# richardbaihe/a3t

Hardware: AMD Instinct MI355X
Metric: mel-frames/sec (train) (higher is better)
Workload: dtype bf16; 1 GPU; VCTK A3T masked-mel train step: 6+6 Conformer blocks d=384 H=2 ff=1536(k3), B=32/GPU, T_mel=1000, T_phn=120, postnet 5x256x5, fwd+bwd+clip+Adam, dropout 0.2/0.2/0.2 + postnet 0.5 (recipe); global_batch=32, parallelism=dp1, params=100799808

## Files before the change

a3t_amd/_lib.py:

```python
import ctypes
import os
from ctypes import POINTER, c_char_p, c_float, c_int, c_int32, c_int64, c_void_p

import torch

HERE = os.path.dirname(os.path.abspath(__file__))
LIB_PATH = os.environ.get("A3T_LIB_PATH") or os.path.join(HERE, "lib", "liba3t_hip.so")

F32, BF16 = 0, 1
ACT_NONE, ACT_RELU, ACT_TANH, ACT_SWISH = 0, 1, 2, 3
ACC_STORE, ACC_ADD, ACC_ATOMIC, ACC_SOLE = 0, 1, 2, 3


class GemmDesc(ctypes.Structure):
    _fields_ = [
        ("A", c_void_p), ("B", c_void_p), ("C", c_void_p), ("bias", c_void_p), ("R", c_void_p), ("S", c_void_p),
        ("M", c_int32), ("N", c_int32), ("K", c_int32),
        ("a_rs", c_int64), ("a_cs", c_int64),
        ("b_rs", c_int64), ("b_cs", c_int64), ("b_ts", c_int64),
        ("c_rs", c_int64),
        ("batch", c_int32), ("batch_inner", c_int32),
        ("a_bs0", c_int64), ("a_bs1", c_int64), ("b_bs0", c_int64), ("b_bs1", c_int64),
        ("c_bs0", c_int64), ("c_bs1", c_int64),
        ("taps", c_int32), ("pad", c_int32), ("dil", c_int32), ("Tseq", c_int32), ("kshift", c_int32),
        ("alpha", c_float),
        ("act", c_int32), ("accumulate", c_int32), ("splitk", c_int32),
        ("a_dtype", c_int32), ("b_dtype", c_int32), ("c_dtype", c_int32), ("compute", c_int32),
        ("s_dtype", c_int32), ("colsum_slots", c_int32),
        ("colsum", c_void_p), ("colsum_bs1", c_int64), ("colsum_scale", c_float), ("drop_key", ctypes.c_uint32),
        ("drop_p", c_float), ("colsum_ss", c_int32),
        ("keep_out", c_void_p), ("keep_in", c_void_p),
        ("a_signmask", c_int32), ("keep_layout", c_int32),
        ("A2", c_void_p), ("B2", c_void_p), ("b2_cs", c_int64), ("b2_bs0", c_int64), ("b2_bs1", c_int64), ("colsum2", c_void_p),
        ("a2_rs", c_int64), ("a_unaligned", c_int32),
    ]


_P = c_void_p
_SIGS = {
    "a3t_gemm": [POINTER(GemmDesc), _P],
    "a3t_gemm_plan": [POINTER(GemmDesc), c_char_p, c_int],
    "a3t_layernorm_fwd": [_P, _P, _P, _P, c_int, _P, _P, c_int, c_int, c_float, _P],
    "a3t_layernorm_bwd": [_P, c_int, _P, _P, _P, _P, _P, _P, _P, _P, _P, _P, c_float, c_int, c_int, c_float,
                          ctypes.c_uint32, _P],
    "a3t_col_reduce": [_P, c_int, _P, _P, _P, _P, c_int, c_int, c_int64, c_int, _P],
    "a3t_f64_to_f32_add": [_P, _P, c_int, c_float, _P],
    "a3t_bn_act_fwd": [_P, _P, _P, _P, _P, _P, _P, _P, _P, c_int, c_int, c_int, c_float, c_float, c_int, c_int, _P],
    "a3t_bn_act_bwd_a": [_P, c_int, _P, _P, _P, _P, _P, _P, c_int, c_int, c_int, _P],
    "a3t_bn_act_bwd_b": [_P, c_int, _P, _P, _P, _P, _P, _P, _P, _P, _P, c_int, c_int, c_int, c_int, _P],
    "a3t_glu_dwconv_fwd": [_P, c_int, _P, _P, _P, c_int, _P, c_int, c_int, c_int, c_int, _P],
    "a3t_glu_dwconv_bwd": [_P, _P, c_int, _P, c_int, _P, _P, c_int, _P, _P, _P, c_int, c_int, c_int, c_int, _P],
    "a3t_add_pos_bias": [_P, _P, _P, _P, _P, c_int, c_int, c_int, _P],
    "a3t_add_pos_bias_bwd": [_P, _P, _P, c_int, c_int, c_int, _P],
    "a3t_relpos_softmax_fwd": [_P, _P, c_int, _P, _P, c_int, c_int, c_int, c_int, c_int64, c_int64, c_int64, c_float, _P,
                               c_float, ctypes.c_uint32, _P],
    "a3t_relpos_softmax_bwd": [_P, c_int, _P, c_int, _P, _P, c_int, c_int, c_int, c_int, c_int64, c_int64, c_int64, c_float, _P,
                               c_float, c_int64, c_int64, ctypes.c_uint32, _P, _P],
    "a3t_attn_fwd_train": [_P, _P, _P, _P, _P, _P, _P, _P, _P, _P, _P, c_int, c_int, c_int, c_int, c_int64, c_int64, c_int64,
                           c_int64, c_float, c_float, ctypes.c_uint32, _P, _P, _P],
    "a3t_attn_scale_rows": [_P, _P, _P, c_int, c_int, c_int, c_int, _P],
    "a3t_attn_bwd_ds": [_P, _P, _P, _P, _P, _P, _P, c_int, c_int, c_int, c_int, c_int64, c_int64, c_int64, c_int64, c_float,
                        c_float, ctypes.c_uint32, c_int, c_int64, _P],
    "a3t_attn_fwd": [_P, _P, _P, _P, _P, _P, _P, _P, c_int, c_int, c_int, c_int, c_int64, c_int64, c_int64, c_int64,
                     c_float, c_float, ctypes.c_uint32, _P, _P, _P],
    "a3t_pwg_block": [_P, _P, _P, _P, _P, _P, _P, _P, c_int, c_int, c_int, _P],
    "a3t_mask_fill": [_P, _P, _P, _P, c_int, c_int, c_int, _P],
    "a3t_embed_finish_fwd": [_P, _P, _P, _P, _P, _P, _P, c_int, c_int, c_int, c_int, c_float, c_float, ctypes.c_uint32,
                             _P, _P],
    "a3t_embed_finish_bwd": [_P, _P, _P, _P, _P, _P, _P, _P, c_int, c_int, c_int, c_int, c_int, c_int, c_float, c_float,
                             ctypes.c_uint32, _P],
    "a3t_scale": [_P, _P, c_int64, c_float, _P],
    "a3t_axpy": [_P, _P, c_int64, c_float, _P],
    "a3t_attn_bias_fold": [_P, c_int32, c_int32, _P, _P, _P, _P],
    "a3t_scale_dev": [_P, _P, c_int64, _P, _P],
    "a3t_slice_rows": [_P, _P, c_int, c_int, c_int, c_int, c_int, c_int, _P],
    "a3t_cast_bf16": [_P, _P, c_int64, _P],
    "a3t_cast_bf16_conv_t": [_P, _P, _P, _P, c_int, c_int, c_int, c_int, _P],
    "a3t_split_bf16": [_P, _P, _P, c_int64, _P],
    "a3t_reflect_pad": [_P, _P, c_int, c_int, c_int, c_int, _P],
    "a3t_stft_amp": [_P, _P, c_int64, c_int, c_int, _P],
    "a3t_logmel_finish": [_P, _P, c_int, c_int, c_int, _P],
    "a3t_mlm_loss": [_P, _P, _P, _P, _P, _P, _P, _P, c_int, c_int, c_int, c_float, _P],
    "a3t_mlm_loss_scratch_floats": [c_int],
    "a3t_sumsq": [_P, c_int64, _P, _P],
# ... 68 lines not shown
```

a3t_amd/build.py:

```python
import os
import subprocess
import sys
from concurrent.futures import ThreadPoolExecutor

HERE = os.path.dirname(os.path.abspath(__file__))
CSRC = os.path.join(HERE, "csrc")
LIBDIR = os.path.join(HERE, "lib")
LIB = os.path.join(LIBDIR, "liba3t_hip.so")
SOURCES = ["gemm.hip", "gemm_bf16.hip", "gemm_bf16_8p.hip", "gemm_bf16_pn.hip", "gemm_bf16_tt.hip", "attn_fused.hip", "norm_reduce.hip", "convmod_attn.hip", "dwconv_vec.hip", "misc.hip", "pwg_fused.hip", "features.hip", "duration.hip"]
FLAGS = ["--offload-arch=gfx950", "-O3", "-std=c++17", "-fPIC", "-ffp-contract=off"] + os.environ.get("A3T_EXTRA_FLAGS", "").split()


RES_SOURCES = ("gemm_bf16.hip", "gemm_bf16_8p.hip", "gemm_bf16_pn.hip", "gemm_bf16_tt.hip", "attn_fused.hip", "norm_reduce.hip")
RES_FLAG = ["-Rpass-analysis=kernel-resource-usage"]


def _save_resources(report, path):
    import json
    import re
    cur, rows = None, {}
    for ln in report.splitlines():
        m = re.search(r"Function Name: (\S+)", ln)
        if m:
            cur = m.group(1)
            rows[cur] = {}
            continue
        m = re.search(r"remark:\s+([\w \[\]/]+?): (\d+)", ln)
        if m and cur:
            rows[cur][m.group(1).strip()] = int(m.group(2))
    with open(path, "w") as f:
        json.dump(rows, f, indent=1)


def _hipcc():
    for c in ("/opt/rocm/bin/hipcc", "hipcc"):
        if os.path.exists(c) or c == "hipcc":
            return c


def _stale(out, deps):
    if not os.path.exists(out):
        return True
    t = os.path.getmtime(out)
    return any(os.path.getmtime(d) > t for d in deps)


# ... 34 lines not shown
```

a3t_amd/csrc/convmod_attn.hip:

```cpp
#include <hip/hip_runtime.h>
#include <stdint.h>
#include "../../include/a3t_hip.h"
#include "dtype_io.h"

#define WAVE 64
__device__ __forceinline__ float sigm(float v) { return 1.f / (1.f + __expf(-v)); }
__device__ __forceinline__ float bf2f_(unsigned int h) { return __uint_as_float(h << 16); }
__device__ __forceinline__ float wsum(float v) {
#pragma unroll
    for (int o = 32; o > 0; o >>= 1) v += __shfl_xor(v, o, WAVE);
    return v;
}
__device__ __forceinline__ float wmax(float v) {
#pragma unroll
    for (int o = 32; o > 0; o >>= 1) v = fmaxf(v, __shfl_xor(v, o, WAVE));
    return v;
}

#define DW_TT 64
#define DW_KMAX 31

template <int KT>
__global__ __launch_bounds__(256) void glu_dwconv_fwd_kernel(const void* __restrict__ g, int g_dt,
                                                             const float* __restrict__ wdw,
// ... 33 lines not shown
    for (int k = 0; k < KT; ++k) w[k] = (k < K) ? wdw[(int64_t)c * K + k] : 0.f;
    const float bias = bdw[c];
    if (K == KT) {
        for (int r0 = ty * 4; r0 < DW_TT; r0 += 16) {
            float v[KT + 3];
#pragma unroll
            for (int j = 0; j < KT + 3; ++j) v[j] = win[r0 + j][tx];
#pragma unroll
            for (int tt = 0; tt < 4; ++tt) {
                float acc = bias;
#pragma unroll
                for (int k = 0; k < KT; ++k) acc += w[k] * v[tt + k];
                int t = t0 + r0 + tt;
                if (t < Tseq) z[(mbase + t) * (int64_t)C + c] = acc;
            }
        }
        return;
    }
    for (int r = ty; r < DW_TT; r += 4) {
        int t = t0 + r;
        if (t >= Tseq) break;
        float acc = bias;
#pragma unroll
        for (int k = 0; k < KT; ++k)
            if (k < K) acc += w[k] * win[r + k][tx];
        z[(mbase + t) * (int64_t)C + c] = acc;
    }
}

int a3t_glu_dwconv_fwd_vec(const void* g, const float* wdw, const float* bdw, void* glu, float* z, int M, int C, int K,
                           int Tseq, hipStream_t stream);
int a3t_glu_dwconv_bwd_vec(const float* dz, const void* g, const void* glu, const float* wdw, void* dg, float* dwdw,
                           float* dbdw, float* dg_colsum, int M, int C, int K, int Tseq, hipStream_t stream);
static inline bool dw_al16(const void* p) { return ((uintptr_t)p & 15) == 0; }

extern "C" int a3t_glu_dwconv_fwd(const void* g, int g_dtype, const float* wdw, const float* bdw, void* glu,
                                  int glu_dtype, float* z, int M, int C, int K, int Tseq, void* stream) {
    if (K > DW_KMAX || (K & 1) == 0 || Tseq <= 0 || M % Tseq) return A3T_EINVAL;
    if (g_dtype == A3T_BF16 && glu_dtype == A3T_BF16 && C % 64 == 0 && dw_al16(g) && dw_al16(glu) && dw_al16(z))
        return a3t_glu_dwconv_fwd_vec(g, wdw, bdw, glu, z, M, C, K, Tseq, (hipStream_t)stream);
    int B = M / Tseq, tiles_t = (Tseq + DW_TT - 1) / DW_TT;
    dim3 grid((C + 63) / 64, B * tiles_t);
    if (K <= 7)
        hipLaunchKernelGGL(glu_dwconv_fwd_kernel<7>, grid, dim3(256), 0, (hipStream_t)stream, g, g_dtype, wdw, bdw, glu,
                           glu_dtype, z, C, K, Tseq, tiles_t);
    else if (K <= 15)
        hipLaunchKernelGGL(glu_dwconv_fwd_kernel<15>, grid, dim3(256), 0, (hipStream_t)stream, g, g_dtype, wdw, bdw, glu,
                           glu_dtype, z, C, K, Tseq, tiles_t);
    else
        hipLaunchKernelGGL(glu_dwconv_fwd_kernel<DW_KMAX>, grid, dim3(256), 0, (hipStream_t)stream, g, g_dtype, wdw, bdw,
                           glu, glu_dtype, z, C, K, Tseq, tiles_t);
    return (int)hipGetLastError();
}

template <int KT>
__global__ __launch_bounds__(256, 3) void glu_dwconv_bwd_kernel(const float* __restrict__ dz, const void* __restrict__ g,
                                                             int g_dt, const void* __restrict__ glu, int glu_dt,
                                                             const float* __restrict__ wdw, void* __restrict__ dg,
                                                             int dg_dt, float* dwdw, float* dbdw, float* dgsum, int C,
                                                             int K, int Tseq, int tiles_t, int tiles_per_block,
                                                             int chunks) {
    __shared__ float wdz[DW_TT + DW_KMAX - 1][64];
    __shared__ float wgl[DW_TT + DW_KMAX - 1][64];
    __shared__ float red[4][64];
    const int tx = threadIdx.x & 63, ty = threadIdx.x >> 6;
    const int c = blockIdx.x * 64 + tx;
// ... 134 lines not shown
        red[ty][tx] = sgb;
        __syncthreads();
        if (ty == 0 && c < C) atomicAdd(&dgsum[C + c], red[0][tx] + red[1][tx] + red[2][tx] + red[3][tx]);
    }
}

extern "C" int a3t_glu_dwconv_bwd(const float* dz, const void* g, int g_dtype, const void* glu, int glu_dtype,
                                  const float* wdw, void* dg, int dg_dtype, float* dwdw, float* dbdw, float* dg_colsum,
                                  int M, int C, int K, int Tseq, void* stream) {
    if (K > DW_KMAX || (K & 1) == 0 || Tseq <= 0 || M % Tseq) return A3T_EINVAL;
    if (g_dtype == A3T_BF16 && glu_dtype == A3T_BF16 && dg_dtype == A3T_BF16 && C % 64 == 0 && dw_al16(g) &&
        dw_al16(glu) && dw_al16(dg) && dw_al16(dz))
        return a3t_glu_dwconv_bwd_vec(dz, g, glu, wdw, dg, dwdw, dbdw, dg_colsum, M, C, K, Tseq, (hipStream_t)stream);
    int B = M / Tseq, tiles_t = (Tseq + DW_TT - 1) / DW_TT;
    int cb = (C + 63) / 64;
    int chunks = 1;
    while (cb * B * chunks < 1024 && chunks < tiles_t) ++chunks;
    int tpb = (tiles_t + chunks - 1) / chunks;
    chunks = (tiles_t + tpb - 1) / tpb;
    dim3 grid(cb, B * chunks);
#define DWB(KT)                                                                                                       \
    hipLaunchKernelGGL(glu_dwconv_bwd_kernel<KT>, grid, dim3(256), 0, (hipStream_t)stream, dz, g, g_dtype, glu, glu_dtype, \
                       wdw, dg, dg_dtype, dwdw, dbdw, dg_colsum, C, K, Tseq, tiles_t, tpb, chunks)
    if (K <= 7)
        DWB(7);
    else if (K <= 15)
        DWB(15);
    else
        DWB(DW_KMAX);
#undef DWB
    return (int)hipGetLastError();
}

__global__ void add_pos_bias_kernel(const void* __restrict__ qkv, const float* __restrict__ bu,
                                    const float* __restrict__ bv, void* __restrict__ qu, void* __restrict__ qv,
                                    int dt, int64_t n, int d) {
    for (int64_t i = (int64_t)blockIdx.x * blockDim.x + threadIdx.x; i < n; i += (int64_t)gridDim.x * blockDim.x) {
        int64_t m = i / d;
        int c = (int)(i - m * d);
        float q = ldx(qkv, dt, m * 3 * d + c);
        stx(qu, dt, i, q + bu[c]);
        stx(qv, dt, i, q + bv[c]);
    }
}
__device__ __forceinline__ void apb_unpack8(const uint4& u, float* f) {
    f[0] = bf2f_(u.x & 0xffff), f[1] = bf2f_(u.x >> 16), f[2] = bf2f_(u.y & 0xffff), f[3] = bf2f_(u.y >> 16);
    f[4] = bf2f_(u.z & 0xffff), f[5] = bf2f_(u.z >> 16), f[6] = bf2f_(u.w & 0xffff), f[7] = bf2f_(u.w >> 16);
}
__device__ __forceinline__ uint4 apb_pack8(const float* f) {
    uint4 u;
    u.x = io_pack2(f[0], f[1]), u.y = io_pack2(f[2], f[3]);
    u.z = io_pack2(f[4], f[5]), u.w = io_pack2(f[6], f[7]);
    return u;
}
__global__ void add_pos_bias_bf16_kernel(const unsigned short* __restrict__ qkv, const float* __restrict__ bu,
                                         const float* __restrict__ bv, unsigned short* __restrict__ qu,
                                         unsigned short* __restrict__ qv, int64_t n8, int d8) {
    for (int64_t i = (int64_t)blockIdx.x * blockDim.x + threadIdx.x; i < n8; i += (int64_t)gridDim.x * blockDim.x) {
        const int64_t m = i / d8;
        const int c = (int)(i - m * d8) * 8;
        float q[8], o[8];
        apb_unpack8(*(const uint4*)(qkv + m * 3 * d8 * 8 + c), q);
        const float4 u0 = *(const float4*)(bu + c), u1 = *(const float4*)(bu + c + 4);
        const float4 v0 = *(const float4*)(bv + c), v1 = *(const float4*)(bv + c + 4);
        const float uu[8] = {u0.x, u0.y, u0.z, u0.w, u1.x, u1.y, u1.z, u1.w};
        const float vv[8] = {v0.x, v0.y, v0.z, v0.w, v1.x, v1.y, v1.z, v1.w};
// ... 468 lines not shown
```

a3t_amd/csrc/dwconv_vec.hip:

```cpp
#include <hip/hip_runtime.h>
#include <stdint.h>
#include "../../include/a3t_hip.h"
#include "dtype_io.h"

#define DW_TT 64
#define DW_KMAX 31
typedef unsigned short u16;

__device__ __forceinline__ float dv_sigm(float v) { return 1.f / (1.f + __expf(-v)); }
__device__ __forceinline__ float dv_bf(unsigned int h) { return __uint_as_float(h << 16); }
__device__ __forceinline__ void dv_unpack8(const uint4& u, float* f) {
    f[0] = dv_bf(u.x & 0xffff), f[1] = dv_bf(u.x >> 16), f[2] = dv_bf(u.y & 0xffff), f[3] = dv_bf(u.y >> 16);
    f[4] = dv_bf(u.z & 0xffff), f[5] = dv_bf(u.z >> 16), f[6] = dv_bf(u.w & 0xffff), f[7] = dv_bf(u.w >> 16);
}
__device__ __forceinline__ uint4 dv_pack8(const float* f) {
    uint4 u;
    u.x = io_pack2(f[0], f[1]), u.y = io_pack2(f[2], f[3]);
    u.z = io_pack2(f[4], f[5]), u.w = io_pack2(f[6], f[7]);
    return u;
}

template <int KT>
__global__ __launch_bounds__(256) void glu_dwconv_fwd_vec_kernel(const u16* __restrict__ g, const float* __restrict__ wdw,
                                                                 const float* __restrict__ bdw, u16* __restrict__ glu,
// ... 59 lines not shown
            for (int k = 0; k < KT; ++k)
                if (k < K) acc += w[k] * win[r + k][tx];
            zt[r][tx] = acc;
        }
    }
    __syncthreads();
    {
        const int rr = tid >> 4, c4 = (tid & 15) * 4;
#pragma unroll
        for (int ps = 0; ps < 4; ++ps) {
            const int r = ps * 16 + rr, t = t0 + r;
            if (t < Tseq) *(float4*)(z + (mbase + t) * (int64_t)C + cblk + c4) = *(const float4*)&zt[r][c4];
        }
    }
}

int a3t_glu_dwconv_fwd_vec(const void* g, const float* wdw, const float* bdw, void* glu, float* z, int M, int C, int K,
                           int Tseq, hipStream_t stream) {
    const int B = M / Tseq, tiles_t = (Tseq + DW_TT - 1) / DW_TT;
    dim3 grid(C / 64, B * tiles_t);
#define DWF(KT)                                                                                                         \
    hipLaunchKernelGGL(glu_dwconv_fwd_vec_kernel<KT>, grid, dim3(256), 0, stream, (const u16*)g, wdw, bdw, (u16*)glu, z, \
                       C, K, Tseq, tiles_t)
    if (K <= 7)
        DWF(7);
    else if (K <= 15)
        DWF(15);
    else
        DWF(DW_KMAX);
#undef DWF
    return (int)hipGetLastError();
}

template <int KT>
__global__ __launch_bounds__(256, 3) void glu_dwconv_bwd_vec_kernel(const float* __restrict__ dz, const u16* __restrict__ g,
                                                                    const u16* __restrict__ glu,
                                                                    const float* __restrict__ wdw, u16* __restrict__ dg,
                                                                    float* dwdw, float* dbdw, float* dgsum, int C, int K,
                                                                    int Tseq, int tiles_t, int tiles_per_block,
                                                                    int chunks) {
    __shared__ __attribute__((aligned(16))) float wdz[DW_TT + DW_KMAX - 1][64];
    __shared__ __attribute__((aligned(16))) u16 wgl[DW_TT + DW_KMAX - 1][64];
    __shared__ __attribute__((aligned(16))) u16 gt[2][DW_TT][64];
    __shared__ float red[4][64];
    const int tid = threadIdx.x, tx = tid & 63, ty = tid >> 6;
    const int cblk = blockIdx.x * 64, c = cblk + tx;
    const int b = blockIdx.y / chunks, tile0 = (blockIdx.y % chunks) * tiles_per_block;
    const int pad = (K - 1) / 2;
    const int64_t mbase = (int64_t)b * Tseq;
    const int rows = DW_TT + K - 1;
    float w[KT], dw[KT];
#pragma unroll
    for (int k = 0; k < KT; ++k) {
        w[k] = (k < K) ? wdw[(int64_t)c * K + k] : 0.f;
        dw[k] = 0.f;
    }
    float db = 0.f, sga = 0.f, sgb = 0.f;
    for (int tile = tile0; tile < min(tiles_t, tile0 + tiles_per_block); ++tile) {
        const int t0 = tile * DW_TT;
        __syncthreads();
        {
            const int r16 = tid >> 4, c4 = (tid & 15) * 4;
            const int r32 = tid >> 3, c8 = (tid & 7) * 8;
            float4 vz[6];
            uint4 vg[3], va[2], vb[2];
#pragma unroll
            for (int ps = 0; ps < 6; ++ps) {
                const int r = ps * 16 + r16, t = t0 - pad + r;
                const bool ok = (r < rows) && (t >= 0) && (t < Tseq);
                vz[ps] = *(const float4*)(dz + (ok ? (mbase + t) * (int64_t)C + cblk + c4 : 0));
                if (!ok) vz[ps] = make_float4(0.f, 0.f, 0.f, 0.f);
            }
#pragma unroll
            for (int ps = 0; ps < 3; ++ps) {
                const int r = ps * 32 + r32, t = t0 - pad + r;
                const bool ok = (r < rows) && (t >= 0) && (t < Tseq);
                vg[ps] = *(const uint4*)(glu + (ok ? (mbase + t) * (int64_t)C + cblk + c8 : 0));
                if (!ok) vg[ps] = make_uint4(0, 0, 0, 0);
            }
#pragma unroll
            for (int ps = 0; ps < 2; ++ps) {
                const int r = ps * 32 + r32, t = t0 + r;
                const bool ok = t < Tseq;
                const u16* src = g + (ok ? (mbase + t) * (int64_t)(2 * C) + cblk + c8 : 0);
                va[ps] = *(const uint4*)src;
                vb[ps] = *(const uint4*)(src + (ok ? C : 0));
            }
#pragma unroll
            for (int ps = 0; ps < 6; ++ps) {
                const int r = ps * 16 + r16;
                if (r < rows) *(float4*)&wdz[r][c4] = vz[ps];
            }
#pragma unroll
            for (int ps = 0; ps < 3; ++ps) {
// ... 75 lines not shown
                if (t < Tseq) {
                    u16* dst = dg + (mbase + t) * (int64_t)(2 * C) + cblk + c8;
                    *(uint4*)dst = *(const uint4*)&gt[0][r][c8];
                    *(uint4*)(dst + C) = *(const uint4*)&gt[1][r][c8];
                }
            }
        }
    }
    __syncthreads();
    float* part = &wdz[0][0];
    for (int i = tid; i < 64 * K; i += 256) part[i] = 0.f;
    __syncthreads();
#pragma unroll
    for (int k = 0; k < KT; ++k)
        if (k < K) atomicAdd(&part[tx * K + k], dw[k]);
    __syncthreads();
    for (int i = tid; i < 64 * K; i += 256) atomicAdd(&dwdw[(int64_t)cblk * K + i], part[i]);
    __syncthreads();
    red[ty][tx] = db;
    __syncthreads();
    if (ty == 0) atomicAdd(&dbdw[c], red[0][tx] + red[1][tx] + red[2][tx] + red[3][tx]);
    if (dgsum) {
        __syncthreads();
        red[ty][tx] = sga;
        __syncthreads();
        if (ty == 0) atomicAdd(&dgsum[c], red[0][tx] + red[1][tx] + red[2][tx] + red[3][tx]);
        __syncthreads();
        red[ty][tx] = sgb;
        __syncthreads();
        if (ty == 0) atomicAdd(&dgsum[C + c], red[0][tx] + red[1][tx] + red[2][tx] + red[3][tx]);
    }
}

int a3t_glu_dwconv_bwd_vec(const float* dz, const void* g, const void* glu, const float* wdw, void* dg, float* dwdw,
                           float* dbdw, float* dg_colsum, int M, int C, int K, int Tseq, hipStream_t stream) {
    const int B = M / Tseq, tiles_t = (Tseq + DW_TT - 1) / DW_TT;
    const int cb = C / 64;
    int chunks = 1;
    while (cb * B * chunks < 640 && chunks < tiles_t) ++chunks;
    const int tpb = (tiles_t + chunks - 1) / chunks;
    chunks = (tiles_t + tpb - 1) / tpb;
    dim3 grid(cb, B * chunks);
#define DWB(KT)                                                                                                       \
    hipLaunchKernelGGL(glu_dwconv_bwd_vec_kernel<KT>, grid, dim3(256), 0, stream, dz, (const u16*)g, (const u16*)glu, \
                       wdw, (u16*)dg, dwdw, dbdw, dg_colsum, C, K, Tseq, tiles_t, tpb, chunks)
    if (K <= 7)
        DWB(7);
    else if (K <= 15)
        DWB(15);
    else
        DWB(DW_KMAX);
#undef DWB
    return (int)hipGetLastError();
}
```

a3t_amd/engine.py:

```python
import math
import os
import zlib
from typing import Dict

import torch

from . import ops
from ._lib import ACC_ADD, ACC_ATOMIC, ACC_STORE, ACT_NONE, ACT_RELU, ACT_SWISH, ACT_TANH, BF16, F32
from .config import A3TConfig
from .params import ParamStore


def legacy_pe_table(c: A3TConfig) -> torch.Tensor:
    d = c.adim
    position = torch.arange(c.max_len - 1, -1, -1.0, dtype=torch.float32).unsqueeze(1)
    div = torch.exp(torch.arange(0, d, 2, dtype=torch.float32) * -(math.log(10000.0) / d))
    pe = torch.zeros(c.max_len, d)
    pe[:, 0::2] = torch.sin(position * div)
    pe[:, 1::2] = torch.cos(position * div)
    return pe


_STREAMS = {}

# ... 95 lines not shown
        self.c = cfg
        self.dropping = bool(dropout and training)
        self.step_seed = 0
        self.store = store
        self.dev = store.device
        self.ws = Workspace(self.dev)
        self.bf16 = (compute == "bf16")
        self.adt = torch.bfloat16 if self.bf16 else torch.float32
        self.cmp = BF16 if self.bf16 else F32
        self.training = training
        self.pe = legacy_pe_table(cfg).to(self.dev)
        self.sv = {}
        self.scratch64 = torch.zeros(4 * max(cfg.ff, 3 * cfg.adim, cfg.postnet_chans, 64), dtype=torch.float64,
                                     device=self.dev)
        self.bn_momentum = 0.1
        self.side = self.side2 = None
        if self.dev.type == "cuda" and os.environ.get("A3T_SIDE_STREAM", "1") != "0":
            self.side = shared_stream(self.dev, "side")
            self.side2 = (shared_stream(self.dev, "side2", high=True)
                          if os.environ.get("A3T_SIDE2", "1") != "0" else self.side)
        self._owned = {}
        self._par = 0
        self._depth = max(2, int(os.environ.get("A3T_SIDE_DEPTH", "48")))
        self._side_ev = [None] * self._depth
        self._wg_group = 4 if (self.bf16 and self.side is not None and self._depth >= 8 and
                               os.environ.get("A3T_WGRAD_GROUP", "1") != "0") else 1
        self._wg_pending = []
        self._wg_slots = set()
        self._gm_ready = None
        self._arena = {k: dict(buf=None, used=0, slots={}, dtype=dt) for k, dt in
                       (("fwd64", torch.float64), ("bwd64", torch.float64), ("bwd32", torch.float32))}
        self.colsum_slots = 16
        self.fuse_ln_dropout = True
        self.post_f32_first = os.environ.get("A3T_POST_F32_FIRST", "1") != "0"
        self.sfc_f32 = True
        self.attn_regen = True
        self.attn_bwd_ds = os.environ.get("A3T_ATTN_BWD_DS", "1") != "0"
        self.attn_signed = os.environ.get("A3T_ATTN_SIGNED", "1") != "0"
        self.attn_dq_dual = os.environ.get("A3T_ATTN_DQ_DUAL", "1") != "0"
        self.attn_dbd_view = os.environ.get("A3T_ATTN_DBD_VIEW", "1") != "0"
        self.attn_dk_main = os.environ.get("A3T_ATTN_DK_MAIN", "1") != "0"
        fa = os.environ.get("A3T_FUSED_ATTN", "auto")
        if fa not in ("auto", "fwd", "0"):
            raise ValueError(f"A3T_FUSED_ATTN={fa!r}: expected auto, fwd or 0 (the flash backward behind '1' left the library in "
                             "round 5, tools/experiments/attn_flash_backward.patch)")
        self.fused_attn_fwd_only = self.bf16 and fa == "fwd"
        self.fused_attn_auto = self.bf16 and fa == "auto"
        self.fused_attn_train = self.bf16 and fa == "auto" and os.environ.get("A3T_FUSED_ATTN_TRAIN", "1") != "0"
        self.fused_attn_train_min = 1 if os.environ.get("A3T_FUSED_ATTN_TRAIN", "1") == "2" else 64
        self._fused_now = False
        self._fused_train_now = False
        self._need_grad = training
        self._mode_tag = None
        if self.bf16:
            for n, v in (("adim", cfg.adim), ("ff", cfg.ff), ("idim", cfg.idim), ("odim", cfg.odim),
                         ("dk", cfg.dk), ("postnet_chans", cfg.postnet_chans or 8)):
                if v % 8:
                    raise ValueError(f"compute='bf16' needs {n} % 8 == 0 (16-byte DMA granules), got {v}")
            self.flat16 = torch.zeros(store.total, dtype=torch.bfloat16, device=self.dev)
            self.p16 = {k: self.flat16[o:o + math.prod(s)].view(s) for k, (o, s) in store.offsets.items()}
        self._ffn_plans = {}
        self._lin_plans = {}
        self._wt = {}
        self._late_cast = self._pos_ahead = True
        self._P_ahead, self._pos_ev = {}, None
        self._cast_ev = self._wt_ev = None
# ... 521 lines not shown
        sums = self._arena_slot("bwd64", tag + ".bnsums", 2 * C)
        ops.bn_act_bwd(dy, z, mean, rstd, p[pre + ".g"], p[pre + ".b"], sums, dz, gr[pre + ".g"], gr[pre + ".b"],
                       self.training, act, zero=False)

    def _conv_fwd(self, tag, pre, x, T):
        p, c = self.store.p, self.c
        M, d = x.shape
        cmp = self.cmp
        y = self._ln_fwd(tag + ".ln", x, pre + ".ln")
        g2 = self._act(tag + ".g", (M, 2 * d))
        ops.linear_fwd(y, self.W(pre + ".pw1"), g2, bias=p[pre + ".pb1"], compute=cmp)
        glu = self._act(tag + ".glu", (M, d))
        z = self.ws.get(tag + ".z", (M, d))
        ops.glu_dwconv_fwd(g2, p[pre + ".dw"], p[pre + ".db"], glu, z, T)
        s = self._act(tag + ".s", (M, d))
        self._bn_fwd(tag, z, pre + ".bn", pre + ".bn", ACT_SWISH, s)
        xo = self.ws.get(tag + ".xo", (M, d))
        ops.linear_fwd(s, self.W(pre + ".pw2"), xo, bias=p[pre + ".pb2"], R=x, compute=cmp,
                       drop=self._drop(c.dropout_rate, tag + ".o"))
        self.sv[tag] = (y, g2, glu, s)
        return xo

    def _conv_bwd(self, tag, pre, g, T, nb=None, nxt=None):
        p, gr, c = self.store.p, self.store.g, self.c
        M, d = g.shape
        cmp = self.cmp
        y, g2, glu, s = self.sv[tag]
        self._sub_begin()
        g16 = self._g16(g)
        ga = self._gm(g, tag + ".o", c.dropout_rate, gr[pre + ".pb2"], 1.0)
        self._lin_wgrad(ga, s, gr[pre + ".pw2"])
        ds = self.ws.get("tmp.ds", (M, d))
        self._lin_dgrad(ga, pre + ".pw2", ds)
        dz = self.ws.get("tmp.dz", (M, d))
        self._bn_bwd(tag, ds, pre + ".bn", ACT_SWISH, dz)
        dg = self._act(self._t("tmp.dg"), (M, 2 * d))
        ops.glu_dwconv_bwd(dz, g2, glu, p[pre + ".dw"], dg, gr[pre + ".dw"], gr[pre + ".db"], T,
                           dgsum=gr[pre + ".pb1"])
        self._lin_wgrad(dg, y, gr[pre + ".pw1"])
        dy = self._act("tmp.dy", (M, d))
        self._lin_dgrad(dg, pre + ".pw1", dy)
        self._pre_ln(ga, g, g16)
        self._ln_bwd(tag + ".ln", dy, pre + ".ln", g, g, g16, nb, nxt)
        self._sub_end()
        return g

    def block_fwd(self, pre, x, pos, keymask, B, T):
        x = self._ffn_fwd(pre + ".ffm", pre + ".ffm", x, T)
        x = self._mha_fwd(pre + ".mha", pre + ".mha", x, pos, keymask, B, T)
        x = self._conv_fwd(pre + ".cnv", pre + ".cnv", x, T)
        x = self._ffn_fwd(pre + ".ff", pre + ".ff", x, T)
        return self._ln_fwd(pre + ".fin", x, pre + ".fin.ln", out_dtype=torch.float32)

    def block_bwd(self, pre, g, B, T):
        gr = self.store.g
        self._ln_bwd(pre + ".fin", g, pre + ".fin.ln", None, g, self._g16(g), (gr[pre + ".ff.b2"], 0.5), pre + ".ff.o")
        self._ffn_bwd(pre + ".ff", pre + ".ff", g, T, (gr[pre + ".cnv.pb2"], 1.0), pre + ".cnv.o")
        self._conv_bwd(pre + ".cnv", pre + ".cnv", g, T, (gr[pre + ".mha.bo"], 1.0), pre + ".mha.o")
        self._mha_bwd(pre + ".mha", pre + ".mha", g, B, T, (gr[pre + ".ffm.b2"], 0.5), pre + ".ffm.o")
        self._ffn_bwd(pre + ".ffm", pre + ".ffm", g, T, None)
        return g

    def forward(self, batch: Dict[str, torch.Tensor], need_grad: bool = True, gscale: float = 1.0):
        c, p, ws = self.c, self.store.p, self.ws
        speech = batch["speech"].contiguous()
        B, Tm, idim = speech.shape
        text = batch["text"].contiguous()
        Tp = text.shape[1]
        T = Tm + Tp
        d = c.adim
        if self.bf16 and (T % 8 or Tm % 8):
# ... 229 lines not shown
```

a3t_amd/ops.py:

```python
import ctypes
import os

import torch

from . import _lib as L
from ._lib import ACC_ADD, ACC_ATOMIC, ACC_SOLE, ACC_STORE, ACT_NONE, ACT_RELU, ACT_SWISH, ACT_TANH, BF16, F32

__all__ = ["gemm", "gemm_plan", "linear_fwd", "linear_bwd_data", "linear_bwd_weight", "conv_fwd", "conv_bwd_data",
           "conv_bwd_weight"]


PROFILE = None


def _stream():
    return ctypes.c_void_p(torch.cuda.current_stream().cuda_stream)


def _ptr(t):
    if t is None:
        return None
    return ctypes.c_void_p(t.data_ptr())


# ... 239 lines not shown


def bn_act_fwd(z, stats, g, b, rmean, rvar, mean_out, rstd_out, y, eps, momentum, training, act):
    M, C = z.shape
    L.check(L.load().a3t_bn_act_fwd(_ptr(z), _ptr(stats), _ptr(g), _ptr(b), _ptr(rmean), _ptr(rvar), _ptr(mean_out),
                                    _ptr(rstd_out), _ptr(y), _dt(y), M, C, eps, momentum, int(training), act,
                                    _stream()), "bn_act_fwd")


def bn_act_bwd(dy, z, mean, rstd, g, b, sums, dz, dg, db, training, act, zero=True):
    M, C = z.shape
    lib = L.load()
    if zero:
        sums.zero_()
    L.check(lib.a3t_bn_act_bwd_a(_ptr(dy), _dt(dy), _ptr(z), _ptr(mean), _ptr(rstd), _ptr(g), _ptr(b), _ptr(sums), M, C,
                                 act, _stream()), "bn_bwd_a")
    L.check(lib.a3t_bn_act_bwd_b(_ptr(dy), _dt(dy), _ptr(z), _ptr(mean), _ptr(rstd), _ptr(g), _ptr(b), _ptr(sums),
                                 _ptr(dz), _ptr(dg), _ptr(db), M, C, int(training), act, _stream()), "bn_bwd_b")


def glu_dwconv_fwd(g, wdw, bdw, glu, z, Tseq):
    M, C = glu.shape
    L.check(L.load().a3t_glu_dwconv_fwd(_ptr(g), _dt(g), _ptr(wdw), _ptr(bdw), _ptr(glu), _dt(glu), _ptr(z), M, C,
                                        wdw.shape[1], Tseq, _stream()), "glu_dwconv_fwd")


def glu_dwconv_bwd(dz, g, glu, wdw, dg, dwdw, dbdw, Tseq, dgsum=None):
    M, C = glu.shape
    L.check(L.load().a3t_glu_dwconv_bwd(_ptr(dz), _ptr(g), _dt(g), _ptr(glu), _dt(glu), _ptr(wdw), _ptr(dg), _dt(dg),
                                        _ptr(dwdw), _ptr(dbdw), _ptr(dgsum), M, C, wdw.shape[1], Tseq, _stream()),
            "glu_dwconv_bwd")


def add_pos_bias(qkv, u, v, qu, qv):
    M, d = qu.shape
    L.check(L.load().a3t_add_pos_bias(_ptr(qkv), _ptr(u), _ptr(v), _ptr(qu), _ptr(qv), _dt(qkv), M, d, _stream()),
            "pos_bias")


def add_pos_bias_bwd(dqu, dqv, dqkv):
    M, d = dqu.shape
    L.check(L.load().a3t_add_pos_bias_bwd(_ptr(dqu), _ptr(dqv), _ptr(dqkv), _dt(dqu), M, d, _stream()),
            "pos_bias_bwd")


def relpos_softmax_fwd(ac, bd, keymask, probs, B, H, T, scale, probs_drop=None, drop=(0.0, 0)):
    L.check(L.load().a3t_relpos_softmax_fwd(_ptr(ac), _ptr(bd), _dt(ac), _ptr(keymask), _ptr(probs), _dt(probs), B, H, T,
                                            T * T, T * T, T * T, scale, _ptr(probs_drop), drop[0], drop[1],
                                            _stream()), "softmax_fwd")


def relpos_softmax_bwd(probs, dprobs, ds, dbd, B, H, T, scale, probs_drop=None, drop_p=0.0, dbd_head_major=False,
                       drop_key=0, rowscale=None):
    bsb, bsh = (T * T, B * T * T) if dbd_head_major else (0, 0)
    L.check(L.load().a3t_relpos_softmax_bwd(_ptr(probs), _dt(probs), _ptr(dprobs), _dt(dprobs), _ptr(ds), _ptr(dbd), _dt(dbd), B, H,
                                            T, T * T, T * T, T * T, scale, _ptr(probs_drop), drop_p, bsb, bsh, drop_key,
                                            _ptr(rowscale), _stream()), "softmax_bwd")


def attn_fused_supported(dk, T):
    return dk % 32 == 0 and dk <= 192 and dk != 160 and T % 8 == 0 and 8 <= T <= 4096


def _attn_q_operands(qu, qv, qkv, pos_bias):
    d = qkv.shape[1] // 3
    if pos_bias is None:
# ... 246 lines not shown
```

include/a3t_hip.h:

```cpp
#ifndef A3T_HIP_H
#define A3T_HIP_H
#include <stdint.h>

#ifdef __cplusplus
extern "C" {
#endif

#define A3T_F32 0
#define A3T_BF16 1

#define A3T_EINVAL (-22)

#define A3T_ACT_NONE 0
#define A3T_ACT_RELU 1
#define A3T_ACT_TANH 2
#define A3T_ACT_SWISH 3

#define A3T_ACC_STORE 0
#define A3T_ACC_ADD 1
#define A3T_ACC_ATOMIC 2
#define A3T_ACC_SOLE 3

typedef struct a3t_gemm_desc {
    const void* A;
// ... 37 lines not shown

int a3t_gemm(const a3t_gemm_desc* d, void* stream);
int a3t_gemm_plan(const a3t_gemm_desc* d, char* name, int len);
int a3t_gemm_8p_supported(int M, int N, int K, int taps, int flags);
int64_t a3t_gemm_keep_bytes(int M, int N);
int a3t_gemm_pn_supported(int M, int N, int K, int taps, int flags);
int a3t_gemm_tt_supported(int M, int N, int K, int batch);

int a3t_layernorm_fwd(const float* x, const float* gamma, const float* beta, void* y, int y_dtype,
                      float* mean, float* rstd, int M, int D, float eps, void* stream);
int a3t_layernorm_bwd(const void* dy, int dy_dtype, const float* x, const float* gamma, const float* mean,
                      const float* rstd, const float* dres, float* dx, void* dx_bf16, float* dgamma,
                      float* dbeta, float* dx_colsum, float dx_colsum_scale, int M, int D, float drop_p,
                      uint32_t drop_key, void* stream);

int a3t_col_reduce(const void* x, int x_dtype, const float* y, const uint8_t* rowmask, double* out0,
                   double* out1, int M, int C, int64_t ld, int mode, void* stream);
int a3t_f64_to_f32_add(const double* src, float* dst, int n, float scale, void* stream);

int a3t_bn_act_fwd(const float* z, const double* stats, const float* gamma, const float* beta,
                   float* running_mean, float* running_var, float* mean_out, float* rstd_out, void* y,
                   int y_dtype, int M, int C, float eps, float momentum, int training, int act, void* stream);
int a3t_bn_act_bwd_a(const void* dy, int dy_dtype, const float* z, const float* mean, const float* rstd,
                     const float* gamma, const float* beta, double* sums, int M, int C, int act, void* stream);
int a3t_bn_act_bwd_b(const void* dy, int dy_dtype, const float* z, const float* mean, const float* rstd,
                     const float* gamma, const float* beta, const double* sums, float* dz, float* dgamma,
                     float* dbeta, int M, int C, int training, int act, void* stream);

int a3t_glu_dwconv_fwd(const void* g, int g_dtype, const float* wdw, const float* bdw, void* glu,
                       int glu_dtype, float* z, int M, int C, int K, int Tseq, void* stream);
int a3t_glu_dwconv_bwd(const float* dz, const void* g, int g_dtype, const void* glu, int glu_dtype,
                       const float* wdw, void* dg, int dg_dtype, float* dwdw, float* dbdw, float* dg_colsum,
                       int M, int C, int K, int Tseq, void* stream);

int a3t_add_pos_bias(const void* qkv, const float* bias_u, const float* bias_v, void* qu, void* qv, int dtype,
                     int M, int d, void* stream);
int a3t_add_pos_bias_bwd(const void* dqu, const void* dqv, void* dqkv, int dtype, int M, int d, void* stream);
int a3t_relpos_softmax_fwd(const void* ac, const void* bd, int scores_dtype, const uint8_t* keymask, void* probs,
                           int probs_dtype, int B, int H, int T, int64_t ac_bs, int64_t bd_bs, int64_t p_bs,
                           float scale, void* probs_drop, float drop_p, uint32_t drop_key, void* stream);
int a3t_relpos_softmax_bwd(const void* probs, int probs_dtype, const void* dprobs, int dprobs_dtype, void* ds,
                           void* dbd, int out_dtype, int B, int H, int T, int64_t p_bs, int64_t dp_bs, int64_t o_bs,
                           float scale, const void* probs_drop, float drop_p, int64_t dbd_bs_b, int64_t dbd_bs_h,
                           uint32_t drop_key, const float* rowscale, void* stream);

int a3t_attn_fwd(const void* qu, const void* qv, const void* k, const void* v, const void* pos, const uint8_t* keymask,
                 void* ctx, float* lse, int B, int H, int T, int dk, int64_t ldq, int64_t ldkv, int64_t ldp, int64_t ldo,
                 float scale, float drop_p, uint32_t drop_key, const float* bias_u, const float* bias_v, void* stream);

int a3t_attn_fwd_train(const void* qu, const void* qv, const void* k, const void* v, const void* pos,
                       const uint8_t* keymask, void* ctx, float* lse, void* probs, void* probs_drop, float* rowscale,
                       int B, int H, int T, int dk, int64_t ldq, int64_t ldkv, int64_t ldp, int64_t ldo, float scale,
                       float drop_p, uint32_t drop_key, const float* bias_u, const float* bias_v, void* stream);
int a3t_attn_scale_rows(const void* x, const float* rowscale, void* y, int B, int H, int T, int dk, void* stream);
int a3t_attn_bwd_ds(const void* dctx, const void* ctx, const void* v, const void* probs, const float* rowscale, void* ds,
                    void* dbd, int B, int H, int T, int dk, int64_t ldo, int64_t ldkv, int64_t dbd_bsb, int64_t dbd_bsh,
                    float scale, float drop_p, uint32_t drop_key, int signed_probs, int64_t ds_bs, void* stream);

int a3t_mask_fill(const float* speech, const uint8_t* masked, const float* mask_feature, void* out,
                  int out_dtype, int M, int C, void* stream);
int a3t_embed_finish_fwd(const float* e, const float* emb, const float* seg, const int64_t* text,
                         const int64_t* spos, const int64_t* tpos, float* xs, int B, int Tm, int Tp, int D,
                         float xscale, float drop_p, uint32_t drop_key, const float* spk, void* stream);
int a3t_embed_finish_bwd(const float* dxs, const float* e, const int64_t* text, const int64_t* spos,
                         const int64_t* tpos, float* de, float* demb, float* dseg, int B, int Tm, int Tp,
                         int D, int V, int nseg, float xscale, float drop_p, uint32_t drop_key, void* stream);
// ... 79 lines not shown
```

Measured before the change: 808,500 mel-frames/s.

## Fuse BatchNorm-swish backward elementwise pass into GLU depthwise-conv backward kernel

The second phase of the conv-module BatchNorm+swish backward, which produced dz, is folded into the tile-load stage of the vectorized GLU/depthwise-conv backward kernel. The kernel now reads ds and z directly, applies the BN/swish gradient in registers using precomputed column sums, and writes dgamma/dbeta from one block row. This drops a full fp32 M×C write and re-read of dz plus one kernel launch per conformer block. In exchange it adds register pressure and extra loads inside the dwconv tile loop, and it keeps the separate column-reduction pass.

```diff
diff --git a/a3t_amd/_lib.py b/a3t_amd/_lib.py
--- a/a3t_amd/_lib.py
+++ b/a3t_amd/_lib.py
@@ -50,6 +50,8 @@
     "a3t_bn_act_bwd_b": [_P, c_int, _P, _P, _P, _P, _P, _P, _P, _P, _P, c_int, c_int, c_int, c_int, _P],
     "a3t_glu_dwconv_fwd": [_P, c_int, _P, _P, _P, c_int, _P, c_int, c_int, c_int, c_int, _P],
     "a3t_glu_dwconv_bwd": [_P, _P, c_int, _P, c_int, _P, _P, c_int, _P, _P, _P, c_int, c_int, c_int, c_int, _P],
+    "a3t_glu_dwconv_bwd_bn": [_P, _P, _P, _P, _P, _P, _P, _P, _P, c_int, c_int, _P, c_int, _P, c_int, _P, _P, c_int, _P, _P, _P,
+                              c_int, c_int, c_int, c_int, _P],
     "a3t_add_pos_bias": [_P, _P, _P, _P, _P, c_int, c_int, c_int, _P],
     "a3t_add_pos_bias_bwd": [_P, _P, _P, c_int, c_int, c_int, _P],
     "a3t_relpos_softmax_fwd": [_P, _P, c_int, _P, _P, c_int, c_int, c_int, c_int, c_int64, c_int64, c_int64, c_float, _P,
diff --git a/a3t_amd/build.py b/a3t_amd/build.py
--- a/a3t_amd/build.py
+++ b/a3t_amd/build.py
@@ -11,7 +11,7 @@
 FLAGS = ["--offload-arch=gfx950", "-O3", "-std=c++17", "-fPIC", "-ffp-contract=off"] + os.environ.get("A3T_EXTRA_FLAGS", "").split()
 
 
-RES_SOURCES = ("gemm_bf16.hip", "gemm_bf16_8p.hip", "gemm_bf16_pn.hip", "gemm_bf16_tt.hip", "attn_fused.hip", "norm_reduce.hip")
+RES_SOURCES = ("gemm_bf16.hip", "gemm_bf16_8p.hip", "gemm_bf16_pn.hip", "gemm_bf16_tt.hip", "attn_fused.hip", "norm_reduce.hip", "dwconv_vec.hip")
 RES_FLAG = ["-Rpass-analysis=kernel-resource-usage"]
 
 
diff --git a/a3t_amd/csrc/convmod_attn.hip b/a3t_amd/csrc/convmod_attn.hip
--- a/a3t_amd/csrc/convmod_attn.hip
+++ b/a3t_amd/csrc/convmod_attn.hip
@@ -89,6 +89,10 @@
                            int Tseq, hipStream_t stream);
 int a3t_glu_dwconv_bwd_vec(const float* dz, const void* g, const void* glu, const float* wdw, void* dg, float* dwdw,
                            float* dbdw, float* dg_colsum, int M, int C, int K, int Tseq, hipStream_t stream);
+int a3t_glu_dwconv_bwd_bn_vec(const float* ds, const float* z, const float* mean, const float* rstd, const float* gamma,
+                              const float* beta, const double* sums, float* dgamma, float* dbeta, int training,
+                              const void* g, const void* glu, const float* wdw, void* dg, float* dwdw, float* dbdw,
+                              float* dg_colsum, int M, int C, int K, int Tseq, hipStream_t stream);
 static inline bool dw_al16(const void* p) { return ((uintptr_t)p & 15) == 0; }
 
 extern "C" int a3t_glu_dwconv_fwd(const void* g, int g_dtype, const float* wdw, const float* bdw, void* glu,
@@ -289,6 +293,21 @@
     return (int)hipGetLastError();
 }
 
+extern "C" int a3t_glu_dwconv_bwd_bn(const float* ds, const float* z, const float* mean, const float* rstd,
+                                     const float* gamma, const float* beta, const double* sums, float* dgamma,
+                                     float* dbeta, int training, int act, const void* g, int g_dtype, const void* glu,
+                                     int glu_dtype, const float* wdw, void* dg, int dg_dtype, float* dwdw, float* dbdw,
+                                     float* dg_colsum, int M, int C, int K, int Tseq, void* stream) {
+    if (K > DW_KMAX || (K & 1) == 0 || Tseq <= 0 || M <= 0 || M % Tseq) return A3T_EINVAL;
+    if (!ds || !z || !mean || !rstd || !gamma || !beta || !sums || !dgamma || !dbeta || act != A3T_ACT_SWISH) return A3T_EINVAL;
+    if (!(g_dtype == A3T_BF16 && glu_dtype == A3T_BF16 && dg_dtype == A3T_BF16 && C > 0 && C % 64 == 0 && dw_al16(g) &&
+          dw_al16(glu) && dw_al16(dg) && dw_al16(ds) && dw_al16(z) && dw_al16(mean) && dw_al16(rstd) && dw_al16(gamma) &&
+          dw_al16(beta)))
+        return A3T_EINVAL;
+    return a3t_glu_dwconv_bwd_bn_vec(ds, z, mean, rstd, gamma, beta, sums, dgamma, dbeta, training, g, glu, wdw, dg, dwdw,
+                                     dbdw, dg_colsum, M, C, K, Tseq, (hipStream_t)stream);
+}
+
 __global__ void add_pos_bias_kernel(const void* __restrict__ qkv, const float* __restrict__ bu,
                                     const float* __restrict__ bv, void* __restrict__ qu, void* __restrict__ qv,
                                     int dt, int64_t n, int d) {
diff --git a/a3t_amd/csrc/dwconv_vec.hip b/a3t_amd/csrc/dwconv_vec.hip
--- a/a3t_amd/csrc/dwconv_vec.hip
+++ b/a3t_amd/csrc/dwconv_vec.hip
@@ -115,13 +115,29 @@
     return (int)hipGetLastError();
 }
 
-template <int KT>
-__global__ __launch_bounds__(256, 3) void glu_dwconv_bwd_vec_kernel(const float* __restrict__ dz, const u16* __restrict__ g,
-                                                                    const u16* __restrict__ glu,
-                                                                    const float* __restrict__ wdw, u16* __restrict__ dg,
-                                                                    float* dwdw, float* dbdw, float* dgsum, int C, int K,
-                                                                    int Tseq, int tiles_t, int tiles_per_block,
-                                                                    int chunks) {
+struct dv_bn_args {
+    const float* ds;
+    const float* z;
+    const float *mean, *rstd, *gamma, *beta;
+    const double* sums;
+    float *dgamma, *dbeta;
+    int M;
+};
+template <bool TRAIN>
+__device__ __forceinline__ float dv_bn_dz(float d, float zv, float mu, float rs, float g, float b, float c0, float c1) {
+    const float zh = (zv - mu) * rs;
+    const float bn = zh * g + b, sg = dv_sigm(bn);
+    d = d * sg * (1.f + bn * (1.f - sg));
+    if (TRAIN) d = d - c0 - zh * c1;
+    return g * rs * d;
+}
+
+template <int KT, int BN>
+__device__ __forceinline__ void glu_dwconv_bwd_vec_body(const float* __restrict__ dz, const dv_bn_args& bn,
+                                                        const u16* __restrict__ g, const u16* __restrict__ glu,
+                                                        const float* __restrict__ wdw, u16* __restrict__ dg, float* dwdw,
+                                                        float* dbdw, float* dgsum, int C, int K, int Tseq, int tiles_t,
+                                                        int tiles_per_block, int chunks) {
     __shared__ __attribute__((aligned(16))) float wdz[DW_TT + DW_KMAX - 1][64];
     __shared__ __attribute__((aligned(16))) u16 wgl[DW_TT + DW_KMAX - 1][64];
     __shared__ __attribute__((aligned(16))) u16 gt[2][DW_TT][64];
@@ -139,10 +155,97 @@
         dw[k] = 0.f;
     }
     float db = 0.f, sga = 0.f, sgb = 0.f;
+    if (BN != 0) {
+        if (ty < 2) {
+            const double invM = 1.0 / (double)bn.M;
+            red[ty][tx] = (float)(bn.sums[(int64_t)ty * C + c] * invM);
+        }
+        if (blockIdx.y == 0 && ty == 0) {
+            bn.dgamma[c] += (float)bn.sums[C + c];
+            bn.dbeta[c] += (float)bn.sums[c];
+        }
+    }
     for (int tile = tile0; tile < min(tiles_t, tile0 + tiles_per_block); ++tile) {
         const int t0 = tile * DW_TT;
         __syncthreads();
-        {
+        if (BN != 0) {
+            constexpr bool TWO_ROUNDS = KT > 15;
+            const int r16 = tid >> 4, c4 = (tid & 15) * 4;
+            const int r32 = tid >> 3, c8 = (tid & 7) * 8;
+            const float* dsb = bn.ds + mbase * (int64_t)C + cblk;
+            const float* zb = bn.z + mbase * (int64_t)C + cblk;
+            const u16* glb = glu + mbase * (int64_t)C + cblk;
+            const u16* gb = g + mbase * (int64_t)(2 * C) + cblk;
+            float4 vs[6], vz[6];
+            auto request = [&](const int ps) __attribute__((always_inline)) {
+                const int t = t0 - pad + ps * 16 + r16;
+                const unsigned off = (unsigned)(min(max(t, 0), Tseq - 1) * C + c4);
+                vs[ps] = *(const float4*)(dsb + off);
+                vz[ps] = *(const float4*)(zb + off);
+            };
+            {
+                uint4 vg[3], va[2], vb[2];
+#pragma unroll
+                for (int ps = 0; ps < 3; ++ps) {
+                    const int r = ps * 32 + r32, t = t0 - pad + r;
+                    const bool ok = (r < rows) && (t >= 0) && (t < Tseq);
+                    vg[ps] = *(const uint4*)(glb + (unsigned)(min(max(t, 0), Tseq - 1) * C + c8));
+                    if (!ok) vg[ps] = make_uint4(0, 0, 0, 0);
+                }
+#pragma unroll
+                for (int ps = 0; ps < 2; ++ps) {
+                    const unsigned off = (unsigned)(min(t0 + ps * 32 + r32, Tseq - 1) * 2 * C + c8);
+                    va[ps] = *(const uint4*)(gb + off);
+                    vb[ps] = *(const uint4*)(gb + off + (unsigned)C);
+                }
+#pragma unroll
+                for (int ps = 0; ps < 3; ++ps) request(ps);
+                __builtin_amdgcn_sched_barrier(0);
+#pragma unroll
+                for (int ps = 0; ps < 3; ++ps) {
+                    const int r = ps * 32 + r32;
+                    if (r < rows) *(uint4*)&wgl[r][c8] = vg[ps];
+                }
+#pragma unroll
+                for (int ps = 0; ps < 2; ++ps) {
+                    const int r = ps * 32 + r32;
+                    *(uint4*)&gt[0][r][c8] = va[ps];
+                    *(uint4*)&gt[1][r][c8] = vb[ps];
+                }
+            }
+            __builtin_amdgcn_sched_barrier(0);
+            if (!TWO_ROUNDS) {
+#pragma unroll
+                for (int ps = 3; ps < 6; ++ps) request(ps);
+                __builtin_amdgcn_sched_barrier(0);
+            }
+            int cc = cblk + c4;
+            asm volatile("" : "+v"(cc));
+            const float4 mu = *(const float4*)(bn.mean + cc), rs = *(const float4*)(bn.rstd + cc);
+            const float4 ga = *(const float4*)(bn.gamma + cc), be = *(const float4*)(bn.beta + cc);
+            const float4 c0 = *(const float4*)&red[0][c4], c1 = *(const float4*)&red[1][c4];
+#pragma unroll
+            for (int ps = 0; ps < 6; ++ps) {
+                if (TWO_ROUNDS && ps == 3) {
+#pragma unroll
+                    for (int p2 = 3; p2 < 6; ++p2) request(p2);
+                    __builtin_amdgcn_sched_barrier(0);
+                }
+                const int r = ps * 16 + r16, t = t0 - pad + r;
+                const bool ok = (t >= 0) && (t < Tseq);
+                if (r < rows) {
+                    float4 o = make_float4(0.f, 0.f, 0.f, 0.f);
+                    if (ok) {
+                        o.x = dv_bn_dz<BN == 2>(vs[ps].x, vz[ps].x, mu.x, rs.x, ga.x, be.x, c0.x, c1.x);
+                        o.y = dv_bn_dz<BN == 2>(vs[ps].y, vz[ps].y, mu.y, rs.y, ga.y, be.y, c0.y, c1.y);
+                        o.z = dv_bn_dz<BN == 2>(vs[ps].z, vz[ps].z, mu.z, rs.z, ga.z, be.z, c0.z, c1.z);
+                        o.w = dv_bn_dz<BN == 2>(vs[ps].w, vz[ps].w, mu.w, rs.w, ga.w, be.w, c0.w, c1.w);
+                    }
+                    *(float4*)&wdz[r][c4] = o;
+                }
+                __builtin_amdgcn_sched_barrier(0);
+            }
+        } else {
             const int r16 = tid >> 4, c4 = (tid & 15) * 4;
             const int r32 = tid >> 3, c8 = (tid & 7) * 8;
             float4 vz[6];
@@ -284,8 +387,31 @@
     }
 }
 
-int a3t_glu_dwconv_bwd_vec(const float* dz, const void* g, const void* glu, const float* wdw, void* dg, float* dwdw,
-                           float* dbdw, float* dg_colsum, int M, int C, int K, int Tseq, hipStream_t stream) {
+template <int KT>
+__global__ __launch_bounds__(256, 3) void glu_dwconv_bwd_vec_kernel(const float* __restrict__ dz, const u16* __restrict__ g,
+                                                                    const u16* __restrict__ glu,
+                                                                    const float* __restrict__ wdw, u16* __restrict__ dg,
+                                                                    float* dwdw, float* dbdw, float* dgsum, int C, int K,
+                                                                    int Tseq, int tiles_t, int tiles_per_block,
+                                                                    int chunks) {
+    glu_dwconv_bwd_vec_body<KT, 0>(dz, dv_bn_args{}, g, glu, wdw, dg, dwdw, dbdw, dgsum, C, K, Tseq, tiles_t,
+                                       tiles_per_block, chunks);
+}
+
+template <int KT, bool TRAIN>
+__global__ __launch_bounds__(256, 3) void glu_dwconv_bn_bwd_vec_kernel(const dv_bn_args bn, const u16* __restrict__ g,
+                                                                       const u16* __restrict__ glu,
+                                                                       const float* __restrict__ wdw, u16* __restrict__ dg,
+                                                                       float* dwdw, float* dbdw, float* dgsum, int C, int K,
+                                                                       int Tseq, int tiles_t, int tiles_per_block,
+                                                                       int chunks) {
+    glu_dwconv_bwd_vec_body<KT, TRAIN ? 2 : 1>(nullptr, bn, g, glu, wdw, dg, dwdw, dbdw, dgsum, C, K, Tseq, tiles_t,
+                                               tiles_per_block, chunks);
+}
+
+static int dwconv_bwd_vec_launch(const float* dz, const dv_bn_args& bn, int training, const void* g, const void* glu, const float* wdw,
+                                 void* dg, float* dwdw, float* dbdw, float* dg_colsum, int M, int C, int K, int Tseq,
+                                 hipStream_t stream) {
     const int B = M / Tseq, tiles_t = (Tseq + DW_TT - 1) / DW_TT;
     const int cb = C / 64;
     int chunks = 1;
@@ -293,9 +419,18 @@
     const int tpb = (tiles_t + chunks - 1) / chunks;
     chunks = (tiles_t + tpb - 1) / tpb;
     dim3 grid(cb, B * chunks);
-#define DWB(KT)                                                                                                       \
-    hipLaunchKernelGGL(glu_dwconv_bwd_vec_kernel<KT>, grid, dim3(256), 0, stream, dz, (const u16*)g, (const u16*)glu, \
-                       wdw, (u16*)dg, dwdw, dbdw, dg_colsum, C, K, Tseq, tiles_t, tpb, chunks)
+#define DWB(KT)                                                                                                        \
+    do {                                                                                                               \
+        if (dz)                                                                                                        \
+            hipLaunchKernelGGL(glu_dwconv_bwd_vec_kernel<KT>, grid, dim3(256), 0, stream, dz, (const u16*)g,           \
+                               (const u16*)glu, wdw, (u16*)dg, dwdw, dbdw, dg_colsum, C, K, Tseq, tiles_t, tpb, chunks); \
+        else if (training)                                                                                             \
+            hipLaunchKernelGGL((glu_dwconv_bn_bwd_vec_kernel<KT, true>), grid, dim3(256), 0, stream, bn, (const u16*)g,  \
+                               (const u16*)glu, wdw, (u16*)dg, dwdw, dbdw, dg_colsum, C, K, Tseq, tiles_t, tpb, chunks); \
+        else                                                                                                           \
+            hipLaunchKernelGGL((glu_dwconv_bn_bwd_vec_kernel<KT, false>), grid, dim3(256), 0, stream, bn, (const u16*)g, \
+                               (const u16*)glu, wdw, (u16*)dg, dwdw, dbdw, dg_colsum, C, K, Tseq, tiles_t, tpb, chunks); \
+    } while (0)
     if (K <= 7)
         DWB(7);
     else if (K <= 15)
@@ -305,3 +440,17 @@
 #undef DWB
     return (int)hipGetLastError();
 }
+
+int a3t_glu_dwconv_bwd_vec(const float* dz, const void* g, const void* glu, const float* wdw, void* dg, float* dwdw,
+                           float* dbdw, float* dg_colsum, int M, int C, int K, int Tseq, hipStream_t stream) {
+    return dwconv_bwd_vec_launch(dz, dv_bn_args{}, 0, g, glu, wdw, dg, dwdw, dbdw, dg_colsum, M, C, K, Tseq, stream);
+}
+
+int a3t_glu_dwconv_bwd_bn_vec(const float* ds, const float* z, const float* mean, const float* rstd, const float* gamma,
+                              const float* beta, const double* sums, float* dgamma, float* dbeta, int training,
+                              const void* g, const void* glu, const float* wdw, void* dg, float* dwdw, float* dbdw,
+                              float* dg_colsum, int M, int C, int K, int Tseq, hipStream_t stream) {
+    if ((int64_t)Tseq * 2 * C >= ((int64_t)1 << 31)) return A3T_EINVAL;
+    const dv_bn_args bn{ds, z, mean, rstd, gamma, beta, sums, dgamma, dbeta, M};
+    return dwconv_bwd_vec_launch(nullptr, bn, training, g, glu, wdw, dg, dwdw, dbdw, dg_colsum, M, C, K, Tseq, stream);
+}
diff --git a/a3t_amd/engine.py b/a3t_amd/engine.py
--- a/a3t_amd/engine.py
+++ b/a3t_amd/engine.py
@@ -151,6 +151,7 @@
                        (("fwd64", torch.float64), ("bwd64", torch.float64), ("bwd32", torch.float32))}
         self.colsum_slots = 16
         self.fuse_ln_dropout = True
+        self.fuse_conv_bn = True
         self.post_f32_first = os.environ.get("A3T_POST_F32_FIRST", "1") != "0"
         self.sfc_f32 = True
         self.attn_regen = True
@@ -738,11 +739,20 @@
         self._lin_wgrad(ga, s, gr[pre + ".pw2"])
         ds = self.ws.get("tmp.ds", (M, d))
         self._lin_dgrad(ga, pre + ".pw2", ds)
-        dz = self.ws.get("tmp.dz", (M, d))
-        self._bn_bwd(tag, ds, pre + ".bn", ACT_SWISH, dz)
         dg = self._act(self._t("tmp.dg"), (M, 2 * d))
-        ops.glu_dwconv_bwd(dz, g2, glu, p[pre + ".dw"], dg, gr[pre + ".dw"], gr[pre + ".db"], T,
-                           dgsum=gr[pre + ".pb1"])
+        z, mean, rstd = self.sv[tag + ".bn"]
+        bg, bb = p[pre + ".bn.g"], p[pre + ".bn.b"]
+        if self.fuse_conv_bn and dg.dtype == torch.bfloat16 and \
+                ops.convmod_fused_ok(g2, glu, p[pre + ".dw"], ds, z, mean, rstd, bg, bb) and dg.data_ptr() % 16 == 0:
+            sums = self._arena_slot("bwd64", tag + ".bnsums", 2 * d)
+            ops.glu_dwconv_bwd_bn(ds, z, mean, rstd, bg, bb, sums, gr[pre + ".bn.g"], gr[pre + ".bn.b"], self.training, ACT_SWISH,
+                                  g2, glu, p[pre + ".dw"], dg, gr[pre + ".dw"], gr[pre + ".db"], T, dgsum=gr[pre + ".pb1"],
+                                  zero=False)
+        else:
+            dz = self.ws.get("tmp.dz", (M, d))
+            self._bn_bwd(tag, ds, pre + ".bn", ACT_SWISH, dz)
+            ops.glu_dwconv_bwd(dz, g2, glu, p[pre + ".dw"], dg, gr[pre + ".dw"], gr[pre + ".db"], T,
+                               dgsum=gr[pre + ".pb1"])
         self._lin_wgrad(dg, y, gr[pre + ".pw1"])
         dy = self._act("tmp.dy", (M, d))
         self._lin_dgrad(dg, pre + ".pw1", dy)
diff --git a/a3t_amd/ops.py b/a3t_amd/ops.py
--- a/a3t_amd/ops.py
+++ b/a3t_amd/ops.py
@@ -295,6 +295,26 @@
             "glu_dwconv_bwd")
 
 
+def convmod_fused_ok(g, glu, wdw, *f32):
+    C, K = glu.shape[1], wdw.shape[1]
+    return (g.dtype == torch.bfloat16 and glu.dtype == torch.bfloat16 and C % 64 == 0 and K % 2 == 1 and K <= 31 and
+            all(t.dtype == torch.float32 for t in f32) and all(t.data_ptr() % 16 == 0 for t in (g, glu) + f32))
+
+
+def glu_dwconv_bwd_bn(ds, z, mean, rstd, gamma, beta, sums, dgamma, dbeta, training, act, g, glu, wdw, dg, dwdw, dbdw, Tseq,
+                      dgsum=None, zero=True):
+    M, C = glu.shape
+    lib = L.load()
+    if zero:
+        sums.zero_()
+    L.check(lib.a3t_bn_act_bwd_a(_ptr(ds), _dt(ds), _ptr(z), _ptr(mean), _ptr(rstd), _ptr(gamma), _ptr(beta), _ptr(sums), M,
+                                 C, act, _stream()), "bn_bwd_a")
+    L.check(lib.a3t_glu_dwconv_bwd_bn(_ptr(ds), _ptr(z), _ptr(mean), _ptr(rstd), _ptr(gamma), _ptr(beta), _ptr(sums),
+                                      _ptr(dgamma), _ptr(dbeta), int(training), act, _ptr(g), _dt(g), _ptr(glu), _dt(glu),
+                                      _ptr(wdw), _ptr(dg), _dt(dg), _ptr(dwdw), _ptr(dbdw), _ptr(dgsum), M, C, wdw.shape[1],
+                                      Tseq, _stream()), "glu_dwconv_bwd_bn")
+
+
 def add_pos_bias(qkv, u, v, qu, qv):
     M, d = qu.shape
     L.check(L.load().a3t_add_pos_bias(_ptr(qkv), _ptr(u), _ptr(v), _ptr(qu), _ptr(qv), _dt(qkv), M, d, _stream()),
diff --git a/include/a3t_hip.h b/include/a3t_hip.h
--- a/include/a3t_hip.h
+++ b/include/a3t_hip.h
@@ -93,6 +93,11 @@
 int a3t_glu_dwconv_bwd(const float* dz, const void* g, int g_dtype, const void* glu, int glu_dtype,
                        const float* wdw, void* dg, int dg_dtype, float* dwdw, float* dbdw, float* dg_colsum,
                        int M, int C, int K, int Tseq, void* stream);
+int a3t_glu_dwconv_bwd_bn(const float* ds, const float* z, const float* mean, const float* rstd,
+                          const float* gamma, const float* beta, const double* sums, float* dgamma,
+                          float* dbeta, int training, int act, const void* g, int g_dtype, const void* glu,
+                          int glu_dtype, const float* wdw, void* dg, int dg_dtype, float* dwdw, float* dbdw,
+                          float* dg_colsum, int M, int C, int K, int Tseq, void* stream);
 
 int a3t_add_pos_bias(const void* qkv, const float* bias_u, const float* bias_v, void* qu, void* qv, int dtype,
                      int M, int d, void* stream);
```

Result: no change. 811,400 mel-frames/s, median of 6 (+0.4%).
